# VideoVerses/VideoTuna-dev

Measured on AMD Instinct MI355X. Metric: finetune samples/sec, CogVideoX-2B T2V LoRA 49x480x720 bf16, higher is better.
Workload: dtype bf16; 1 GPU; CogVideoX-2B T2V LoRA finetune 49x480x720 (configs[1]): latents [4,13,16,60,90], text [4,226,4096], r=4 LoRA on to_q/k/v/out, 4 samples per optimizer step as in the YAML (batch_size 2 x accumulate_grad_batches 2), run as 1 micro-batch(es) of 4; mode=lora, model=CogVideoX-2B, micro_batch=4, accumulate_grad_batches=1, global_batch=4, seq_len=17776, layers=30, parallelism=dp1, recompute=none (107 GB of block activations kept in HBM), weights=seeded random init (no checkpoints offline), text=pre-encoded prompt embeddings (synthetic), latents=pre-encoded latents (synthetic)

## Files before the change

videotuna-dev_amd/csrc/attn_fwd.hip:

```cpp
#include "common.h"

struct AttnFwdParams {
    const bf16_t* q;
    const bf16_t* k;
    const bf16_t* v;
    bf16_t* o;
    float* lse2;
    int S, H, B;
    long long q_rs, k_rs, v_rs, o_rs;
    long long q_bs, k_bs, v_bs, o_bs;
    float scale_log2;
    const float* bias_t;
};

#define FQ 128
#define FWD_THREADS 256
#define FK 64
#define NEG_BIG (-1.0e30f)
#define LAZY_THR 8.0f

template <bool PRESCALED, bool BIAS = false>
__global__ __launch_bounds__(FWD_THREADS, 2) void attn_fwd_hd64_kernel(AttnFwdParams p) {
    __shared__ __attribute__((aligned(16))) char smem[32768];
    const int tid = threadIdx.x, lane = tid & 63, wave = tid >> 6;
    const int r = lane & 31, h = lane >> 5;
    const int nqt = (p.S + FQ - 1) / FQ;
    const int id = xcd_remap(blockIdx.x, gridDim.x);
    const int qt = id % nqt;
    const int bh = id / nqt;
    const int head = bh % p.H, b = bh / p.H;
    const int q0 = qt * FQ + wave * 32;

    const bf16_t* qb = p.q + (size_t)b * p.q_bs + head * 64;
    const bf16_t* kb = p.k + (size_t)b * p.k_bs + head * 64;
    const bf16_t* vb = p.v + (size_t)b * p.v_bs + head * 64;
    __amdgpu_buffer_rsrc_t rk = make_rsrc(kb, (unsigned)((long long)(p.S - 1) * p.k_rs * 2 + 128));
    __amdgpu_buffer_rsrc_t rv = make_rsrc(vb, (unsigned)((long long)(p.S - 1) * p.v_rs * 2 + 128));

    bf16x8 qf[4];
    {
        int qrow = q0 + r;
        if (qrow > p.S - 1) qrow = p.S - 1;
        const bf16_t* qp = qb + (size_t)qrow * p.q_rs + 8 * h;
#pragma unroll
        for (int s = 0; s < 4; ++s) qf[s] = *(const bf16x8*)(qp + 16 * s);
    }

    int k_voff[2], v_voff[2], k_lds[2], v_lds[2];
#pragma unroll
    for (int j = 0; j < 2; ++j) {
        int i = tid + FWD_THREADS * j;
        int key = i >> 3, c = i & 7;
        k_voff[j] = (int)(key * p.k_rs * 2) + c * 16;
        v_voff[j] = (int)(key * p.v_rs * 2) + c * 16;
        k_lds[j] = key * 128 + ((c ^ ((key >> 1) & 7)) << 4);
        v_lds[j] = 8192 + key * 128 + ((c ^ (((key >> 1) & 1) << 2)) << 4);
    }
    const int wv = __builtin_amdgcn_readfirstlane(wave);
    constexpr int NPC = 2;
    int kd_voff[2], vd_voff[2];
#pragma unroll
    for (int j = 0; j < NPC; ++j) {
        const int key = 8 * (wv + 4 * j) + (lane >> 3);
        kd_voff[j] = (int)(key * p.k_rs * 2) + (((lane & 7) ^ ((key >> 1) & 7)) << 4);
        vd_voff[j] = (int)(key * p.v_rs * 2) + (((lane & 7) ^ (((key >> 1) & 1) << 2)) << 4);
    }
    auto dma = [&](int t, int buf) {
        const int ks = (int)((long long)t * FK * p.k_rs * 2);
        const int vs = (int)((long long)t * FK * p.v_rs * 2);
#pragma unroll
        for (int j = 0; j < NPC; ++j) {
            char* dst = smem + buf * 16384 + (wv + 4 * j) * 1024;
            __builtin_amdgcn_raw_ptr_buffer_load_lds(rk, (__attribute__((address_space(3))) void*)dst, 16, kd_voff[j], ks, 0, 0);
            __builtin_amdgcn_raw_ptr_buffer_load_lds(rv, (__attribute__((address_space(3))) void*)(dst + 8192), 16, vd_voff[j], vs, 0, 0);
        }
    };

    int kfo[4];
#pragma unroll
    for (int s = 0; s < 4; ++s) kfo[s] = r * 128 + (((2 * s + h) ^ ((r >> 1) & 7)) << 4);
    int vfo[2];
    {
        const int g = lane >> 4;
        const int ql = (lane & 15) >> 2;
        const int pl = lane & 3;
        const int keyl = 4 * (g >> 1) + ql;
        const int x = (ql >> 1) & 1;
#pragma unroll
        for (int dt = 0; dt < 2; ++dt) {
            int chunk = 4 * dt + 2 * (g & 1) + (pl >> 1);
            vfo[dt] = 8192 + keyl * 128 + ((chunk ^ (x << 2)) << 4) + (pl & 1) * 8;
        }
    }

    f32x16 o_acc[2];
#pragma unroll
    for (int i = 0; i < 16; ++i) { o_acc[0][i] = 0.f; o_acc[1][i] = 0.f; }
    float m_run = PRESCALED ? 0.f : NEG_BIG, l_run = 0.f;
    f32x16 negm;
#pragma unroll
    for (int i = 0; i < 16; ++i) negm[i] = 0.f;
    const float sc = p.scale_log2;

    const int nt = (p.S + FK - 1) / FK;
    dma(0, 0);
    __syncthreads();
    for (int t = 0; t < nt; ++t) {
        const int buf = t & 1;
        if (t + 1 < nt) dma(t + 1, buf ^ 1);
        const char* base = smem + buf * 16384;

        f32x16 st[2];
        if constexpr (PRESCALED) {
#pragma unroll
            for (int s = 0; s < 4; ++s) {
#pragma unroll
                for (int kt2 = 0; kt2 < 2; ++kt2) {
                    bf16x8 kf = *(const bf16x8*)(base + kt2 * 4096 + kfo[s]);
                    st[kt2] = __builtin_amdgcn_mfma_f32_32x32x16_bf16(kf, qf[s], s == 0 ? negm : st[kt2], 0, 0, 0);
                }
            }
            if ((t + 1) * FK > p.S) {
#pragma unroll
                for (int kt2 = 0; kt2 < 2; ++kt2)
#pragma unroll
                    for (int i = 0; i < 16; ++i) {
                        int key = t * FK + kt2 * 32 + (i & 3) + 8 * (i >> 2) + 4 * h;
                        if (key >= p.S) st[kt2][i] = NEG_BIG;
                    }
            }
            float mx = st[0][0];
#pragma unroll
            for (int i = 1; i < 16; ++i) mx = fmaxf(mx, st[0][i]);
#pragma unroll
            for (int i = 0; i < 16; ++i) mx = fmaxf(mx, st[1][i]);
            if (t == 0 || !__all(mx <= LAZY_THR)) {
                mx = fmaxf(mx, __shfl_xor(mx, 32, 64));
                const float delta = (t == 0) ? mx : fmaxf(mx, 0.f);
                const float alpha = (t == 0) ? 1.0f : __builtin_amdgcn_exp2f(-delta);
                m_run += delta;
                l_run *= alpha;
#pragma unroll
                for (int i = 0; i < 16; ++i) {
                    o_acc[0][i] *= alpha; o_acc[1][i] *= alpha;
                    st[0][i] -= delta; st[1][i] -= delta;
                    negm[i] = -m_run;
                }
            }
            float psum = 0.f;
#pragma unroll
            for (int kt2 = 0; kt2 < 2; ++kt2)
#pragma unroll
                for (int i = 0; i < 16; ++i) {
                    float pv = __builtin_amdgcn_exp2f(st[kt2][i]);
                    st[kt2][i] = pv;
                    psum += pv;
                }
            l_run += psum;
        } else {
#pragma unroll
        for (int i = 0; i < 16; ++i) { st[0][i] = 0.f; st[1][i] = 0.f; }
#pragma unroll
        for (int s = 0; s < 4; ++s) {
#pragma unroll
            for (int kt2 = 0; kt2 < 2; ++kt2) {
                bf16x8 kf = *(const bf16x8*)(base + kt2 * 4096 + kfo[s]);
                st[kt2] = __builtin_amdgcn_mfma_f32_32x32x16_bf16(kf, qf[s], st[kt2], 0, 0, 0);
            }
        }
        if constexpr (BIAS) {
            int qc = q0 + r;
            qc = qc < p.S ? qc : p.S - 1;
            const float* bp = p.bias_t + ((size_t)head * p.S) * p.S + qc;
            const float isc = 1.0f / sc * 1.4426950408889634f;
#pragma unroll
            for (int kt2 = 0; kt2 < 2; ++kt2)
#pragma unroll
                for (int i = 0; i < 16; ++i) {
                    int key = t * FK + kt2 * 32 + (i & 3) + 8 * (i >> 2) + 4 * h;
                    key = key < p.S ? key : p.S - 1;
                    st[kt2][i] += bp[(size_t)key * p.S] * isc;
                }
        }
        if ((t + 1) * FK > p.S) {
#pragma unroll
            for (int kt2 = 0; kt2 < 2; ++kt2)
#pragma unroll
                for (int i = 0; i < 16; ++i) {
                    int key = t * FK + kt2 * 32 + (i & 3) + 8 * (i >> 2) + 4 * h;
                    if (key >= p.S) st[kt2][i] = NEG_BIG;
                }
        }
        float mx = st[0][0];
#pragma unroll
        for (int i = 1; i < 16; ++i) mx = fmaxf(mx, st[0][i]);
#pragma unroll
        for (int i = 0; i < 16; ++i) mx = fmaxf(mx, st[1][i]);
        mx = fmaxf(mx, __shfl_xor(mx, 32, 64));
        const float m_new = fmaxf(m_run, PRESCALED ? mx : mx * sc);
        const float alpha = __builtin_amdgcn_exp2f(m_run - m_new);
        m_run = m_new;
        float psum = 0.f;
#pragma unroll
        for (int kt2 = 0; kt2 < 2; ++kt2)
#pragma unroll
            for (int i = 0; i < 16; ++i) {
                float pv = __builtin_amdgcn_exp2f(PRESCALED ? st[kt2][i] - m_new : st[kt2][i] * sc - m_new);
                st[kt2][i] = pv;
                psum += pv;
            }
        l_run = l_run * alpha + psum;
#pragma unroll
        for (int i = 0; i < 16; ++i) { o_acc[0][i] *= alpha; o_acc[1][i] *= alpha; }

        }

#pragma unroll
        for (int kt2 = 0; kt2 < 2; ++kt2) {
#pragma unroll
            for (int s2 = 0; s2 < 2; ++s2) {
                bf16x8 pf;
#pragma unroll
                for (int j = 0; j < 8; ++j) pf[j] = (bf16_t)st[kt2][8 * s2 + j];
#pragma unroll
                for (int dt = 0; dt < 2; ++dt) {
                    const char* vp = base + vfo[dt] + (kt2 * 32 + s2 * 16) * 128;
                    short4v lo = __builtin_amdgcn_ds_read_tr16_b64_v4i16((short4v __attribute__((address_space(3)))*)(vp));
                    short4v hi = __builtin_amdgcn_ds_read_tr16_b64_v4i16((short4v __attribute__((address_space(3)))*)(vp + 8 * 128));
                    typedef __attribute__((ext_vector_type(8))) short short8v;
                    short8v v8 = {lo[0], lo[1], lo[2], lo[3], hi[0], hi[1], hi[2], hi[3]};
                    o_acc[dt] = __builtin_amdgcn_mfma_f32_32x32x16_bf16(__builtin_bit_cast(bf16x8, v8), pf, o_acc[dt], 0, 0, 0);
                }
            }
        }
        __syncthreads();
    }

    const float l_tot = l_run + __shfl_xor(l_run, 32, 64);
    const float inv = 1.0f / l_tot;
    const int qrow = q0 + r;
    if (qrow < p.S) {
        bf16_t* op = p.o + (size_t)b * p.o_bs + (size_t)qrow * p.o_rs + head * 64;
#pragma unroll
        for (int dt = 0; dt < 2; ++dt)
#pragma unroll
            for (int g4 = 0; g4 < 4; ++g4) {
                u32x2 w;
                w[0] = pack2(o_acc[dt][4 * g4 + 0] * inv, o_acc[dt][4 * g4 + 1] * inv);
                w[1] = pack2(o_acc[dt][4 * g4 + 2] * inv, o_acc[dt][4 * g4 + 3] * inv);
                *(u32x2*)(op + dt * 32 + 8 * g4 + 4 * h) = w;
            }
        if (h == 0) p.lse2[((size_t)b * p.H + head) * p.S + qrow] = m_run + __builtin_amdgcn_logf(l_tot);
    }
}

__global__ __launch_bounds__(256, 2) void attn_fwd_hd64_m16_kernel(AttnFwdParams p) {
    __shared__ __attribute__((aligned(16))) char smem[32768];
    const int tid = threadIdx.x, lane = tid & 63, wave = tid >> 6;
    const int c = lane & 15, g = lane >> 4, ql = (lane & 15) >> 2, pl = lane & 3;
    const int nqt = (p.S + 127) / 128;
    const int id = xcd_remap(blockIdx.x, gridDim.x);
    const int qtb = id % nqt;
    const int bh = id / nqt;
    const int head = bh % p.H, b = bh / p.H;
    const int q0 = qtb * 128 + wave * 32;

    const bf16_t* qb = p.q + (size_t)b * p.q_bs + head * 64;
    const bf16_t* kb = p.k + (size_t)b * p.k_bs + head * 64;
    const bf16_t* vb = p.v + (size_t)b * p.v_bs + head * 64;
    __amdgpu_buffer_rsrc_t rk = make_rsrc(kb, (unsigned)((long long)(p.S - 1) * p.k_rs * 2 + 128));
    __amdgpu_buffer_rsrc_t rv = make_rsrc(vb, (unsigned)((long long)(p.S - 1) * p.v_rs * 2 + 128));

    bf16x8 qf[2][2];
#pragma unroll
    for (int qt = 0; qt < 2; ++qt) {
        int qrow = q0 + 16 * qt + c;
        if (qrow > p.S - 1) qrow = p.S - 1;
        const bf16_t* qp = qb + (size_t)qrow * p.q_rs + 8 * g;
#pragma unroll
        for (int s = 0; s < 2; ++s) qf[qt][s] = *(const bf16x8*)(qp + 32 * s);
    }
    const int wv = __builtin_amdgcn_readfirstlane(wave);
    int kd_voff[2], vd_voff[2];
#pragma unroll
    for (int j = 0; j < 2; ++j) {
        const int key = 8 * (wv + 4 * j) + (lane >> 3);
        kd_voff[j] = (int)(key * p.k_rs * 2) + (((lane & 7) ^ ((key >> 1) & 7)) << 4);
        vd_voff[j] = (int)(key * p.v_rs * 2) + (((lane & 7) ^ (key & 6)) << 4);
    }
    auto dma = [&](int t, int buf) {
        const int ks = (int)((long long)t * FK * p.k_rs * 2);
        const int vs = (int)((long long)t * FK * p.v_rs * 2);
#pragma unroll
        for (int j = 0; j < 2; ++j) {
            char* dst = smem + buf * 16384 + (wv + 4 * j) * 1024;
            __builtin_amdgcn_raw_ptr_buffer_load_lds(rk, (__attribute__((address_space(3))) void*)dst, 16, kd_voff[j], ks, 0, 0);
            __builtin_amdgcn_raw_ptr_buffer_load_lds(rv, (__attribute__((address_space(3))) void*)(dst + 8192), 16, vd_voff[j], vs, 0, 0);
        }
    };
    int kfo[2];
#pragma unroll
    for (int s = 0; s < 2; ++s) kfo[s] = c * 128 + (((4 * s + g) ^ ((c >> 1) & 7)) << 4);
    int vfo[4];
#pragma unroll
    for (int dt = 0; dt < 4; ++dt) vfo[dt] = 8192 + (4 * g + ql) * 128 + (((2 * dt + (pl >> 1)) ^ ((4 * g + ql) & 6)) << 4) + (pl & 1) * 8;

    f32x4 o16[4][2];
#pragma unroll
    for (int dt = 0; dt < 4; ++dt)
#pragma unroll
        for (int qt = 0; qt < 2; ++qt) o16[dt][qt] = (f32x4){0.f, 0.f, 0.f, 0.f};
    float m_run[2] = {0.f, 0.f}, l_run[2] = {0.f, 0.f};
    f32x4 negm[2] = {{0.f, 0.f, 0.f, 0.f}, {0.f, 0.f, 0.f, 0.f}};
    auto group_max = [&](float x) {
        x = fmaxf(x, __builtin_bit_cast(float, __builtin_amdgcn_ds_swizzle(__builtin_bit_cast(int, x), 0x401F)));
        return fmaxf(x, __shfl_xor(x, 32, 64));
    };

    const int nt = (p.S + FK - 1) / FK;
    dma(0, 0);
    __syncthreads();
    for (int t = 0; t < nt; ++t) {
        const int buf = t & 1;
        if (t + 1 < nt) dma(t + 1, buf ^ 1);
        const char* base = smem + buf * 16384;
        f32x4 st[4][2];
#pragma unroll
        for (int s = 0; s < 2; ++s)
#pragma unroll
            for (int kt = 0; kt < 4; ++kt) {
                const bf16x8 kf = *(const bf16x8*)(base + kt * 2048 + kfo[s]);
#pragma unroll
                for (int qt = 0; qt < 2; ++qt)
                    st[kt][qt] = __builtin_amdgcn_mfma_f32_16x16x32_bf16(kf, qf[qt][s], s == 0 ? negm[qt] : st[kt][qt], 0, 0, 0);
            }
        if ((t + 1) * FK > p.S) {
#pragma unroll
            for (int kt = 0; kt < 4; ++kt)
#pragma unroll
                for (int i = 0; i < 4; ++i)
                    if (t * FK + 16 * kt + 4 * g + i >= p.S) { st[kt][0][i] = NEG_BIG; st[kt][1][i] = NEG_BIG; }
        }
        float mx[2];
#pragma unroll
        for (int qt = 0; qt < 2; ++qt) {
            mx[qt] = st[0][qt][0];
#pragma unroll
            for (int kt = 0; kt < 4; ++kt)
#pragma unroll
                for (int i = 0; i < 4; ++i) mx[qt] = fmaxf(mx[qt], st[kt][qt][i]);
        }
        if (t == 0 || !__all(fmaxf(mx[0], mx[1]) <= LAZY_THR)) {
#pragma unroll
            for (int qt = 0; qt < 2; ++qt) {
                const float mq = group_max(mx[qt]);
                const float delta = (t == 0) ? mq : fmaxf(mq, 0.f);
                const float alpha = (t == 0) ? 1.0f : __builtin_amdgcn_exp2f(-delta);
                m_run[qt] += delta;
                l_run[qt] *= alpha;
#pragma unroll
                for (int dt = 0; dt < 4; ++dt)
#pragma unroll
                    for (int i = 0; i < 4; ++i) o16[dt][qt][i] *= alpha;
#pragma unroll
                for (int kt = 0; kt < 4; ++kt)
#pragma unroll
                    for (int i = 0; i < 4; ++i) st[kt][qt][i] -= delta;
#pragma unroll
                for (int i = 0; i < 4; ++i) negm[qt][i] = -m_run[qt];
            }
        }
#pragma unroll
        for (int qt = 0; qt < 2; ++qt) {
            float psum = 0.f;
#pragma unroll
            for (int kt = 0; kt < 4; ++kt)
#pragma unroll
                for (int i = 0; i < 4; ++i) {
                    const float pv = __builtin_amdgcn_exp2f(st[kt][qt][i]);
                    st[kt][qt][i] = pv;
                    psum += pv;
                }
            l_run[qt] += psum;
        }
#pragma unroll
        for (int s2 = 0; s2 < 2; ++s2) {
            bf16x8 pf[2];
#pragma unroll
            for (int qt = 0; qt < 2; ++qt)
#pragma unroll
                for (int j = 0; j < 4; ++j) { pf[qt][j] = (bf16_t)st[2 * s2][qt][j]; pf[qt][4 + j] = (bf16_t)st[2 * s2 + 1][qt][j]; }
#pragma unroll
            for (int dt = 0; dt < 4; ++dt) {
                const char* vp = base + vfo[dt] + s2 * 4096;
                short4v lo = __builtin_amdgcn_ds_read_tr16_b64_v4i16((short4v __attribute__((address_space(3)))*)(vp));
                short4v hi = __builtin_amdgcn_ds_read_tr16_b64_v4i16((short4v __attribute__((address_space(3)))*)(vp + 2048));
                typedef __attribute__((ext_vector_type(8))) short short8v;
                short8v v8 = {lo[0], lo[1], lo[2], lo[3], hi[0], hi[1], hi[2], hi[3]};
                const bf16x8 vt = __builtin_bit_cast(bf16x8, v8);
#pragma unroll
                for (int qt = 0; qt < 2; ++qt) o16[dt][qt] = __builtin_amdgcn_mfma_f32_16x16x32_bf16(vt, pf[qt], o16[dt][qt], 0, 0, 0);
            }
        }
        __syncthreads();
    }
#pragma unroll
    for (int qt = 0; qt < 2; ++qt) {
        float l_tot = l_run[qt];
        l_tot += __builtin_bit_cast(float, __builtin_amdgcn_ds_swizzle(__builtin_bit_cast(int, l_tot), 0x401F));
        l_tot += __shfl_xor(l_tot, 32, 64);
        const float inv = 1.0f / l_tot;
        const int qrow = q0 + 16 * qt + c;
        if (qrow < p.S) {
            bf16_t* op = p.o + (size_t)b * p.o_bs + (size_t)qrow * p.o_rs + head * 64;
#pragma unroll
            for (int dt = 0; dt < 4; ++dt) {
                u32x2 w;
                w[0] = pack2(o16[dt][qt][0] * inv, o16[dt][qt][1] * inv);
                w[1] = pack2(o16[dt][qt][2] * inv, o16[dt][qt][3] * inv);
                *(u32x2*)(op + 16 * dt + 4 * g) = w;
            }
            if (g == 0) p.lse2[((size_t)b * p.H + head) * p.S + qrow] = m_run[qt] + __builtin_amdgcn_logf(l_tot);
        }
    }
}

extern "C" int vt_attn_fwd_hd64(const void* q, const void* k, const void* v, void* o, float* lse2,
                                int B, int H, int S,
                                long long q_rs, long long k_rs, long long v_rs, long long o_rs,
                                long long q_bs, long long k_bs, long long v_bs, long long o_bs,
                                float softmax_scale, int q_prescaled, void* stream) {
    if (B <= 0 || H <= 0 || S <= 0) return VT_ERR_BAD_SHAPE;
    if ((q_rs % 8) || (k_rs % 8) || (v_rs % 8) || (o_rs % 4) || (q_bs % 8) || (k_bs % 8) || (v_bs % 8) || (o_bs % 4))
        return VT_ERR_BAD_SHAPE;
    if ((((uintptr_t)q) | ((uintptr_t)k) | ((uintptr_t)v)) & 15) return VT_ERR_BAD_ALIGN;
    if (((uintptr_t)o) & 7) return VT_ERR_BAD_ALIGN;
    if ((long long)S * k_rs * 2 >= 0x7fffffffLL || (long long)S * v_rs * 2 >= 0x7fffffffLL) return VT_ERR_BAD_SHAPE;
    AttnFwdParams p;
    p.q = (const bf16_t*)q; p.k = (const bf16_t*)k; p.v = (const bf16_t*)v; p.o = (bf16_t*)o; p.lse2 = lse2;
    p.S = S; p.H = H; p.B = B;
    p.q_rs = q_rs; p.k_rs = k_rs; p.v_rs = v_rs; p.o_rs = o_rs;
    p.q_bs = q_bs; p.k_bs = k_bs; p.v_bs = v_bs; p.o_bs = o_bs;
    p.scale_log2 = softmax_scale * 1.4426950408889634f;
    p.bias_t = nullptr;
    const int nqt = (S + FQ - 1) / FQ;
    if (q_prescaled == 2)
        hipLaunchKernelGGL(attn_fwd_hd64_m16_kernel, dim3(nqt * H * B), dim3(256), 0, (hipStream_t)stream, p);
    else if (q_prescaled) hipLaunchKernelGGL(attn_fwd_hd64_kernel<true>, dim3(nqt * H * B), dim3(FWD_THREADS), 0, (hipStream_t)stream, p);
    else hipLaunchKernelGGL(attn_fwd_hd64_kernel<false>, dim3(nqt * H * B), dim3(FWD_THREADS), 0, (hipStream_t)stream, p);
    return hipGetLastError() == hipSuccess ? VT_OK : VT_ERR_LAUNCH;
}

extern "C" int vt_attn_fwd_bias_hd64(const void* q, const void* k, const void* v, const float* bias_t, void* o, float* lse2,
                                     int B, int H, int S,
                                     long long q_rs, long long k_rs, long long v_rs, long long o_rs,
                                     long long q_bs, long long k_bs, long long v_bs, long long o_bs,
                                     float softmax_scale, void* stream) {
    if (B <= 0 || H <= 0 || S <= 0 || bias_t == nullptr || lse2 == nullptr || !(softmax_scale > 0.f)) return VT_ERR_BAD_SHAPE;
    if ((q_rs % 8) || (k_rs % 8) || (v_rs % 8) || (o_rs % 4) || (q_bs % 8) || (k_bs % 8) || (v_bs % 8) || (o_bs % 4))
        return VT_ERR_BAD_SHAPE;
    if ((((uintptr_t)q) | ((uintptr_t)k) | ((uintptr_t)v)) & 15) return VT_ERR_BAD_ALIGN;
    if ((((uintptr_t)o) & 7) || (((uintptr_t)bias_t) & 3)) return VT_ERR_BAD_ALIGN;
    if ((long long)S * k_rs * 2 >= 0x7fffffffLL || (long long)S * v_rs * 2 >= 0x7fffffffLL) return VT_ERR_BAD_SHAPE;
    AttnFwdParams p;
    p.q = (const bf16_t*)q; p.k = (const bf16_t*)k; p.v = (const bf16_t*)v; p.o = (bf16_t*)o; p.lse2 = lse2;
    p.S = S; p.H = H; p.B = B;
    p.q_rs = q_rs; p.k_rs = k_rs; p.v_rs = v_rs; p.o_rs = o_rs;
    p.q_bs = q_bs; p.k_bs = k_bs; p.v_bs = v_bs; p.o_bs = o_bs;
    p.scale_log2 = softmax_scale * 1.4426950408889634f;
    p.bias_t = bias_t;
    const int nqt = (S + FQ - 1) / FQ;
    hipLaunchKernelGGL((attn_fwd_hd64_kernel<false, true>), dim3(nqt * H * B), dim3(FWD_THREADS), 0, (hipStream_t)stream, p);
    return hipGetLastError() == hipSuccess ? VT_OK : VT_ERR_LAUNCH;
}
```

Baseline: 2.774 samples/s.

## Peel and unroll prescaled attention forward loop, raise occupancy bound to four

Restructures the forward attention KV loop into an inlined tile lambda with compile-time flags for the first and last tile, peeling tile 0 and unrolling the rest by two with fixed buffer indices. Boundary masking and the first-tile rescale branch are removed from the steady-state loop. Dead offset arrays are dropped so the DMA offsets collapse to one register each. Launch bounds for the prescaled variant go from 2 to 4 blocks per CU. The aim is less VGPR pressure, fewer runtime branches and more latency hiding, at the risk of spills under the tighter register budget and larger code size.

```diff
diff --git a/videotuna-dev_amd/csrc/attn_fwd.hip b/videotuna-dev_amd/csrc/attn_fwd.hip
--- a/videotuna-dev_amd/csrc/attn_fwd.hip
+++ b/videotuna-dev_amd/csrc/attn_fwd.hip
@@ -18,9 +18,10 @@
 #define FK 64
 #define NEG_BIG (-1.0e30f)
 #define LAZY_THR 8.0f
+template <int V> struct IntC { static constexpr int value = V; };
 
 template <bool PRESCALED, bool BIAS = false>
-__global__ __launch_bounds__(FWD_THREADS, 2) void attn_fwd_hd64_kernel(AttnFwdParams p) {
+__global__ __launch_bounds__(FWD_THREADS, PRESCALED ? 4 : 2) void attn_fwd_hd64_kernel(AttnFwdParams p) {
     __shared__ __attribute__((aligned(16))) char smem[32768];
     const int tid = threadIdx.x, lane = tid & 63, wave = tid >> 6;
     const int r = lane & 31, h = lane >> 5;
@@ -46,33 +47,19 @@
         for (int s = 0; s < 4; ++s) qf[s] = *(const bf16x8*)(qp + 16 * s);
     }
 
-    int k_voff[2], v_voff[2], k_lds[2], v_lds[2];
-#pragma unroll
-    for (int j = 0; j < 2; ++j) {
-        int i = tid + FWD_THREADS * j;
-        int key = i >> 3, c = i & 7;
-        k_voff[j] = (int)(key * p.k_rs * 2) + c * 16;
-        v_voff[j] = (int)(key * p.v_rs * 2) + c * 16;
-        k_lds[j] = key * 128 + ((c ^ ((key >> 1) & 7)) << 4);
-        v_lds[j] = 8192 + key * 128 + ((c ^ (((key >> 1) & 1) << 2)) << 4);
-    }
     const int wv = __builtin_amdgcn_readfirstlane(wave);
     constexpr int NPC = 2;
-    int kd_voff[2], vd_voff[2];
-#pragma unroll
-    for (int j = 0; j < NPC; ++j) {
-        const int key = 8 * (wv + 4 * j) + (lane >> 3);
-        kd_voff[j] = (int)(key * p.k_rs * 2) + (((lane & 7) ^ ((key >> 1) & 7)) << 4);
-        vd_voff[j] = (int)(key * p.v_rs * 2) + (((lane & 7) ^ (((key >> 1) & 1) << 2)) << 4);
-    }
+    const int key0 = 8 * wv + (lane >> 3);
+    const int kd_voff = (int)(key0 * p.k_rs * 2) + (((lane & 7) ^ ((key0 >> 1) & 7)) << 4);
+    const int vd_voff = (int)(key0 * p.v_rs * 2) + (((lane & 7) ^ (((key0 >> 1) & 1) << 2)) << 4);
     auto dma = [&](int t, int buf) {
-        const int ks = (int)((long long)t * FK * p.k_rs * 2);
-        const int vs = (int)((long long)t * FK * p.v_rs * 2);
 #pragma unroll
         for (int j = 0; j < NPC; ++j) {
+            const int ks = (int)((long long)(t * FK + 32 * j) * p.k_rs * 2);
+            const int vs = (int)((long long)(t * FK + 32 * j) * p.v_rs * 2);
             char* dst = smem + buf * 16384 + (wv + 4 * j) * 1024;
-            __builtin_amdgcn_raw_ptr_buffer_load_lds(rk, (__attribute__((address_space(3))) void*)dst, 16, kd_voff[j], ks, 0, 0);
-            __builtin_amdgcn_raw_ptr_buffer_load_lds(rv, (__attribute__((address_space(3))) void*)(dst + 8192), 16, vd_voff[j], vs, 0, 0);
+            __builtin_amdgcn_raw_ptr_buffer_load_lds(rk, (__attribute__((address_space(3))) void*)dst, 16, kd_voff, ks, 0, 0);
+            __builtin_amdgcn_raw_ptr_buffer_load_lds(rv, (__attribute__((address_space(3))) void*)(dst + 8192), 16, vd_voff, vs, 0, 0);
         }
     };
 
@@ -103,24 +90,23 @@
     const float sc = p.scale_log2;
 
     const int nt = (p.S + FK - 1) / FK;
-    dma(0, 0);
-    __syncthreads();
-    for (int t = 0; t < nt; ++t) {
-        const int buf = t & 1;
-        if (t + 1 < nt) dma(t + 1, buf ^ 1);
+    auto tile = [&](const int t, const int buf, auto first_c, auto next_c, auto last_c) __attribute__((always_inline)) {
+        constexpr int NEXT = decltype(next_c)::value;
+        constexpr bool FIRST = decltype(first_c)::value, LAST = decltype(last_c)::value;
+        if (NEXT == 1 || (NEXT == 2 && t + 1 < nt)) dma(t + 1, buf ^ 1);
         const char* base = smem + buf * 16384;
 
         f32x16 st[2];
         if constexpr (PRESCALED) {
 #pragma unroll
-            for (int s = 0; s < 4; ++s) {
-#pragma unroll
-                for (int kt2 = 0; kt2 < 2; ++kt2) {
+            for (int kt2 = 0; kt2 < 2; ++kt2) {
+#pragma unroll
+                for (int s = 0; s < 4; ++s) {
                     bf16x8 kf = *(const bf16x8*)(base + kt2 * 4096 + kfo[s]);
                     st[kt2] = __builtin_amdgcn_mfma_f32_32x32x16_bf16(kf, qf[s], s == 0 ? negm : st[kt2], 0, 0, 0);
                 }
             }
-            if ((t + 1) * FK > p.S) {
+            if (LAST && (t + 1) * FK > p.S) {
 #pragma unroll
                 for (int kt2 = 0; kt2 < 2; ++kt2)
 #pragma unroll
@@ -134,10 +120,10 @@
             for (int i = 1; i < 16; ++i) mx = fmaxf(mx, st[0][i]);
 #pragma unroll
             for (int i = 0; i < 16; ++i) mx = fmaxf(mx, st[1][i]);
-            if (t == 0 || !__all(mx <= LAZY_THR)) {
+            if (FIRST || !__all(mx <= LAZY_THR)) {
                 mx = fmaxf(mx, __shfl_xor(mx, 32, 64));
-                const float delta = (t == 0) ? mx : fmaxf(mx, 0.f);
-                const float alpha = (t == 0) ? 1.0f : __builtin_amdgcn_exp2f(-delta);
+                const float delta = FIRST ? mx : fmaxf(mx, 0.f);
+                const float alpha = FIRST ? 1.0f : __builtin_amdgcn_exp2f(-delta);
                 m_run += delta;
                 l_run *= alpha;
 #pragma unroll
@@ -146,15 +132,16 @@
                     st[0][i] -= delta; st[1][i] -= delta;
                     negm[i] = -m_run;
                 }
-            }
-            float psum = 0.f;
+                asm("" : "+v"(negm));
+            }
+            float psum;
 #pragma unroll
             for (int kt2 = 0; kt2 < 2; ++kt2)
 #pragma unroll
                 for (int i = 0; i < 16; ++i) {
                     float pv = __builtin_amdgcn_exp2f(st[kt2][i]);
                     st[kt2][i] = pv;
-                    psum += pv;
+                    psum = (kt2 == 0 && i == 0) ? pv : psum + pv;
                 }
             l_run += psum;
         } else {
@@ -182,7 +169,7 @@
                     st[kt2][i] += bp[(size_t)key * p.S] * isc;
                 }
         }
-        if ((t + 1) * FK > p.S) {
+        if (LAST && (t + 1) * FK > p.S) {
 #pragma unroll
             for (int kt2 = 0; kt2 < 2; ++kt2)
 #pragma unroll
@@ -200,14 +187,14 @@
         const float m_new = fmaxf(m_run, PRESCALED ? mx : mx * sc);
         const float alpha = __builtin_amdgcn_exp2f(m_run - m_new);
         m_run = m_new;
-        float psum = 0.f;
+        float psum;
 #pragma unroll
         for (int kt2 = 0; kt2 < 2; ++kt2)
 #pragma unroll
             for (int i = 0; i < 16; ++i) {
                 float pv = __builtin_amdgcn_exp2f(PRESCALED ? st[kt2][i] - m_new : st[kt2][i] * sc - m_new);
                 st[kt2][i] = pv;
-                psum += pv;
+                psum = (kt2 == 0 && i == 0) ? pv : psum + pv;
             }
         l_run = l_run * alpha + psum;
 #pragma unroll
@@ -234,6 +221,24 @@
             }
         }
         __syncthreads();
+    };
+
+    constexpr IntC<0> c0; constexpr IntC<1> c1; constexpr IntC<2> c2;
+    dma(0, 0);
+    __syncthreads();
+    if constexpr (PRESCALED) {
+        tile(0, 0, c1, c2, c1);
+        int t = 1;
+        for (; t + 2 < nt; t += 2) {
+            tile(t, 1, c0, c1, c0);
+            tile(t + 1, 0, c0, c1, c0);
+        }
+        if (t < nt) {
+            tile(t, 1, c0, c2, c1);
+            if (t + 1 < nt) tile(t + 1, 0, c0, c0, c1);
+        }
+    } else {
+        for (int t = 0; t < nt; ++t) tile(t, t & 1, c0, c2, c1);
     }
 
     const float l_tot = l_run + __shfl_xor(l_run, 32, 64);
```

New measurement: 2.781 samples/s (median of 6 runs). No clear change (+0.2%).
